# LY-zhang-yi-hao/ORB-SLAM3_byZyh

Measured on AMD Instinct MI355X. Metric: ORB features/ms (640x480, 8-level) + LocalBA iter ms @1/2/4/8 GPU, higher is better.
Workload: dtype u8; 1 GPU; C2: batch of 64 synthetic 640x480 frames per GPU, nFeatures=1000, 8 levels, extraction+description (ORBextractor::operator()); frames_per_gpu=64, width=640, height=480, nfeatures=1000, nlevels=8, batches_in_flight=4, parallelism=frame-sharded x1

## Files before the change

orb-slam3_byzyh_amd/csrc/orb_extract.hip:

```cpp
#include <hip/hip_ext.h>
#include <hip/hip_runtime.h>

#include <algorithm>
#include <cstdio>
#include <cstdlib>
#include <cstring>
#include <mutex>
#include <string>
#include <type_traits>
#include <vector>

#include "orb_extract_geom.h"
#include "orb_hd.h"
#include "orb_sincos.h"
#include "orbgpu.h"
#include "orbgpu_internal.h"

using namespace orbgpu;

namespace {

constexpr int kPatternSrc[1024] = {
#include "orb_pattern31.inc"
};
// ... 495 lines not shown
            const int r = r0o + lr;
            if (lr < rpp && r < nrow) {
                const int y = oy0 + r;
                const uint8_t* urow = ubuf + (reflect101(y, A.hl) - uy0) * kPairUP;
                uint8_t* dst = plane_l + (size_t)(y + kEdge) * A.pitch_l;
                const int pc = pc0 + 8 * ch, x = pc - kEdge;
                if (x >= ox0 && x + 8 <= ox1 && x >= 0 && x + 8 <= A.wl) {
                    *reinterpret_cast<unsigned long long*>(dst + pc) = lds_bytes8(urow, x - ux0);
                } else {
#pragma unroll
                    for (int b = 0; b < 8; ++b)
                        if (x + b >= ox0 && x + b < ox1) dst[pc + b] = urow[reflect101(x + b, A.wl) - ux0];
                }
            }
        }
    }
    {
        const int sx = XN.x - ux0, sx1 = min(XN.x + 1, ux0 + uw - 1) - ux0;
        pyr_resize_col<kTileH / 2>(ubuf, &yrowT[r0], sx, sx1, (unsigned)XN.y & 0xffffu, (unsigned)XN.y >> 16,
                                   vxn < A.simd_n, true, &tile[r0][tx], kTileW + 8);
    }
    __syncthreads();
#pragma unroll
    for (int r = tid >> 4; r < kTileH; r += 16) {
        const int c = (tid & 15) * 8;
        const int py = Y0 + r, px = X0 + c;
        if (py < ey && px < ex) {
            uint8_t* dst = plane_n + (size_t)py * A.pitch_n + px;
            if (px + 7 < ex) {
                *reinterpret_cast<unsigned long long*>(dst) = lds_bytes8(tile[r], c);
            } else {
                for (int k = 0; k < 8 && px + k < ex; ++k) dst[k] = tile[r][c + k];
            }
        }
    }
}

__global__ __launch_bounds__(256) void k_debug_blur(const uint8_t* __restrict__ view, int pitch, int w, int h,
                                                    uint8_t* __restrict__ out) {
    const int x = blockIdx.x * 256 + threadIdx.x, y = blockIdx.y;
    if (x >= w) return;
    uint32_t acc = 1u << 15;
    for (int i = 0; i < 7; ++i) {
        const uint8_t* row = view + (size_t)reflect101(y + i - 3, h) * pitch;
        uint32_t hs = 0;
        for (int k = 0; k < 7; ++k) hs += (uint32_t)(blur_tap(k) * row[reflect101(x + k - 3, w)]);
        acc += (uint32_t)blur_tap(i) * hs;
    }
    out[(size_t)y * w + x] = (uint8_t)(acc >> 16);
}

__device__ __forceinline__ u16x2 swap16(u16x2 a) { return __builtin_shufflevector(a, a, 1, 0); }
__device__ __forceinline__ int fast_score(const uint8_t* __restrict__ p, const int (&off)[16]) {
    const int v = p[0];
    const u16x2 vv = w16(v + 256, v + 256);
    u16x2 D[8];
#pragma unroll
    for (int k = 0; k < 8; ++k)
        D[k] = vv - __builtin_bit_cast(u16x2, (uint32_t)p[off[k]] | ((uint32_t)p[off[k + 8]] << 16));
    auto at = [&](const u16x2 (&a)[8], int k) { return k < 8 ? a[k] : swap16(a[k - 8]); };
    u16x2 mn2[8], mx2[8], mn4[8], mx4[8];
#pragma unroll
    for (int k = 0; k < 8; ++k) {
        mn2[k] = __builtin_elementwise_min(D[k], at(D, k + 1));
        mx2[k] = __builtin_elementwise_max(D[k], at(D, k + 1));
    }
#pragma unroll
    for (int k = 0; k < 8; ++k) {
        mn4[k] = __builtin_elementwise_min(mn2[k], at(mn2, k + 2));
        mx4[k] = __builtin_elementwise_max(mx2[k], at(mx2, k + 2));
    }
    u16x2 dark = w16(0, 0), bright = w16(0xffff, 0xffff);
#pragma unroll
    for (int k = 0; k < 8; ++k) {
        const u16x2 mn8 = __builtin_elementwise_min(mn4[k], at(mn4, k + 4));
        const u16x2 mx8 = __builtin_elementwise_max(mx4[k], at(mx4, k + 4));
        dark = __builtin_elementwise_max(dark, __builtin_elementwise_min(mn8, swap16(D[k])));
        bright = __builtin_elementwise_min(bright, __builtin_elementwise_max(mx8, swap16(D[k])));
    }
    const int best_dark = (int)max(dark.x, dark.y) - 256, best_bright = (int)min(bright.x, bright.y) - 256;
    return max(best_dark, -best_bright) - 1;
}

__device__ __forceinline__ bool is_local_max(const uint8_t* __restrict__ sc, int stride, int idx, int s) {
    const uint8_t* q = sc + idx;
    return s > q[-stride - 1] && s > q[-stride] && s > q[-stride + 1] && s > q[-1] && s > q[1] &&
           s > q[stride - 1] && s > q[stride] && s > q[stride + 1];
}

__device__ __forceinline__ uint32_t pack_key(int x, int y, int score) {
    return (uint32_t)score | ((uint32_t)x << 8) | ((uint32_t)y << 20);
}
__device__ __forceinline__ int key_x(uint32_t k) { return (int)((k >> 8) & 0xfff); }
__device__ __forceinline__ int key_y(uint32_t k) { return (int)(k >> 20); }
__device__ __forceinline__ int key_score(uint32_t k) { return (int)(k & 0xff); }

#define FAST_STAMP(k) do { if (stp && lane == 0) stp[k] = __builtin_amdgcn_s_memtime(); } while (0)
template <int kWS, int kSS>
__device__ __forceinline__ void fast_cell(const KernelGeom& g, const CellDesc& C, const LevelGeom& L, int f, int cid,
                                          int lane, uint8_t* win, uint8_t* sc, uint16_t* cl, const uint8_t* src,
                                          int shift, int room, uint32_t* __restrict__ cand, int32_t* __restrict__ cell_count,
                                          uint8_t* __restrict__ cell_thr, unsigned long long* stp) {
    const int ww = C.win_w, wh = C.win_h;
    const int ws = kWS ? kWS : (shift + ww + 3) & ~3, nwr = ws >> 2;
    const int ss = kSS ? kSS : (ww - 4 + 3) & ~3;
    auto sc_at = [&](int e) { return ((e >> 7) - 2) * ss + (e & 127) - 2; };
    const uint32_t* wsrc = reinterpret_cast<const uint32_t*>(src - shift);
    uint32_t* win32 = reinterpret_cast<uint32_t*>(win);
    const int lr = lane >> 4, lw = lane & 15;
    if (nwr <= 16 && wh <= 48) {
        const uintptr_t wb = reinterpret_cast<uintptr_t>(wsrc);
        const uint64_t wbu = (uint64_t)(uint32_t)uniform((int)(uint32_t)wb) | (uint64_t)(uint32_t)uniform((int)(uint32_t)(wb >> 32)) << 32;
        const __amdgpu_buffer_rsrc_t rw = __builtin_amdgcn_make_buffer_rsrc(reinterpret_cast<void*>(wbu), (short)0, uniform(room), kBufDword3);
        const int pitch = uniform(L.pitch);
        const uint32_t vo = (uint32_t)(lr * pitch + 4 * lw);
        uint32_t v[12];
#pragma unroll
        for (int k = 0; k < 12; ++k) v[k] = __builtin_amdgcn_raw_buffer_load_b32(rw, vo, 4 * k * pitch, 0);
#pragma unroll
        for (int k = 0; k < 12; ++k) {
            const int r = 4 * k + lr;
            if (r < wh && lw < nwr) win32[r * nwr + lw] = v[k];
        }
    } else
    for (int w0 = 0; w0 < nwr; w0 += 16) {
        const int w = w0 + lw;
        for (int r0 = 0; r0 < wh; r0 += 16) {
            uint32_t v[4];
#pragma unroll
            for (int k = 0; k < 4; ++k) {
                const int r = r0 + 4 * k + lr;
                v[k] = (r < wh && w < nwr) ? wsrc[(size_t)r * (L.pitch >> 2) + w] : 0u;
            }
#pragma unroll
            for (int k = 0; k < 4; ++k) {
                const int r = r0 + 4 * k + lr;
                if (r < wh && w < nwr) win32[r * nwr + w] = v[k];
            }
        }
    }
    wave_sync();
    FAST_STAMP(1);
    win += shift;
    const int dw = ww - 6, dh = wh - 6;
    const int nd = (dw > 0 && dh > 0) ? dw * dh : 0;
    int off[16];
    {
        const int cx[16] = {0, 1, 2, 3, 3, 3, 2, 1, 0, -1, -2, -3, -3, -3, -2, -1};
        const int cy[16] = {3, 3, 2, 1, 0, -1, -2, -3, -3, -3, -2, -1, 0, 1, 2, 3};
#pragma unroll
        for (int k = 0; k < 16; ++k) off[k] = cx[k] + cy[k] * ws;
    }
    const int ini = g.ini_th, mint = g.min_th;
    int nlist = 0;
    if (nd > 0) {
        const int no = (dw + 7) >> 3, nitems = dh * no;
        const uint32_t* wrow = reinterpret_cast<const uint32_t*>(win - shift);
        const int wsw = ws >> 2;
        const u16x2 tt = w16(mint, mint);
        auto ext8 = [&](const uint32_t* row, int o, int off, uint32_t& a, uint32_t& b) {
            const int d = 2 * o + (off >> 2);
            const uint32_t w0 = row[d], w1 = row[d + 1], w2 = row[d + 2];
            a = __builtin_amdgcn_alignbyte(w1, w0, off & 3);
            b = __builtin_amdgcn_alignbyte(w2, w1, off & 3);
        };
        auto lo16 = [](uint32_t v) { return as_u16x2(__builtin_amdgcn_perm(v, v, 0x0c010c00u)); };
        auto hi16 = [](uint32_t v) { return as_u16x2(__builtin_amdgcn_perm(v, v, 0x0c030c02u)); };
        auto pass2 = [&](u16x2 v, u16x2 p0, u16x2 p4, u16x2 p8, u16x2 p12) {
            const u16x2 bmax = __builtin_elementwise_min(__builtin_elementwise_max(p0, p8), __builtin_elementwise_max(p4, p12));
            const u16x2 dmin = __builtin_elementwise_max(__builtin_elementwise_min(p0, p8), __builtin_elementwise_min(p4, p12));
            const u16x2 m = __builtin_elementwise_max(__builtin_elementwise_sub_sat(bmax, v), __builtin_elementwise_sub_sat(v, dmin));
            uint32_t r;
            asm("v_pk_min_u16 %0, %1, %2" : "=v"(r) : "v"(__builtin_bit_cast(uint32_t, __builtin_elementwise_sub_sat(m, tt))), "v"(0x00010001u));
            return r;
        };
        auto octet_bits = [&](uint32_t C0, uint32_t D0, uint32_t R0, uint32_t U0, uint32_t L0, uint32_t C1,
                              uint32_t D1, uint32_t R1, uint32_t U1, uint32_t L1) {
            const uint32_t p01 = pass2(lo16(C0), lo16(D0), lo16(R0), lo16(U0), lo16(L0));
            const uint32_t p23 = pass2(hi16(C0), hi16(D0), hi16(R0), hi16(U0), hi16(L0));
            const uint32_t p45 = pass2(lo16(C1), lo16(D1), lo16(R1), lo16(U1), lo16(L1));
            const uint32_t p67 = pass2(hi16(C1), hi16(D1), hi16(R1), hi16(U1), hi16(L1));
            const uint32_t t = p01 | (p23 << 2) | (p45 << 4) | (p67 << 6);
            return (t & 0xffu) | (t >> 15);
        };
        int r = lane / no, o = lane - (lane / no) * no;
        const int dr = 64 / no, dq = 64 - dr * no;
        for (int i0 = 0; i0 < nitems; i0 += 64) {
            const int it = i0 + lane;
            unsigned bits = 0;
            if (it < nitems) {
                const uint32_t* rc = wrow + (r + 3) * wsw;
                uint32_t L0, L1, C0, C1, R0, R1, U0, U1, D0, D1;
                ext8(rc, o, shift, L0, L1);
                ext8(rc, o, shift + 3, C0, C1);
                ext8(rc, o, shift + 6, R0, R1);
                ext8(rc - 3 * wsw, o, shift + 3, U0, U1);
                ext8(rc + 3 * wsw, o, shift + 3, D0, D1);
                bits = octet_bits(C0, D0, R0, U0, L0, C1, D1, R1, U1, L1);
                const int rem = dw - 8 * o;
                if (rem < 8) bits &= (1u << rem) - 1u;
            }
            const int row = r, oct = o;
            o += dq;
            r += dr;
            if (o >= no) { o -= no; ++r; }
            const int cnt = __popc(bits);
            const int incl = wave_incl_scan_dpp(cnt);
            int pos = nlist + incl - cnt;
            const int base_idx = ((row + 3) << 7) + 8 * oct + 3;
            while (bits) {
                const int k = __builtin_ctz(bits);
                bits &= bits - 1u;
                cl[pos++] = (uint16_t)(base_idx + k);
            }
            nlist += __builtin_amdgcn_readlane(incl, 63);
        }
    }
    wave_sync();
    FAST_STAMP(2);
    int ncand = 0;
    for (int j0 = 0; j0 < nlist; j0 += 64) {
        const int j = j0 + lane;
        int idx = 0, s = -1;
        if (j < nlist) {
            idx = cl[j];
            s = fast_score(win + (idx >> 7) * ws + (idx & 127), off);
        }
        const bool is_c = s >= mint;
        const unsigned long long m = ballot(is_c);
        if (is_c) {
            cl[ncand + rank_in(m)] = (uint16_t)idx;
            sc[sc_at(idx)] = (uint8_t)min(s, 255);
        }
        ncand += __popcll(m);
    }
    wave_sync();
    FAST_STAMP(3);
    FAST_STAMP(4);
    uint8_t* lmv = win - shift;
    bool any = false;
    for (int j = lane; j < ncand; j += 64) {
        const int si = sc_at(cl[j]), s = sc[si];
        const bool lm = is_local_max(sc, ss, si, s);
        lmv[j] = lm ? (uint8_t)(s + 1) : (uint8_t)0;
        any |= (s >= ini) && lm;
    }
    const int t = ballot(any) ? ini : mint;
    wave_sync();
    FAST_STAMP(5);
    uint32_t* out = cand + (size_t)f * g.cand_frame_cap + L.cand_off + C.slot;
    int count = 0;
    for (int j0 = 0; j0 < ncand; j0 += 64) {
        const int j = j0 + lane;
        bool keep = false;
        int idx = 0, s = 0;
        if (j < ncand) {
            idx = cl[j];
            const int lv = lmv[j];
            s = lv - 1;
            keep = lv > 0 && s >= t;
        }
        const unsigned long long m = ballot(keep);
        if (keep) {
            const int pos = count + rank_in(m);
            const int r = idx >> 7, c = idx & 127;
            if (pos < C.cap) out[pos] = pack_key(C.off_x + c, C.off_y + r, s);
        }
        count += __popcll(m);
    }
    if (lane == 0) {
        cell_count[(size_t)f * g.ncells + cid] = min(count, (int)C.cap);
        cell_thr[(size_t)f * g.ncells + cid] = (uint8_t)t;
    }
    if (stp && lane == 0) { stp[6] = __builtin_amdgcn_s_memtime(); stp[8] = wall_clock64(); stp[9] = nlist; stp[10] = ncand; }
}


__global__ __launch_bounds__(256) void k_fast_cells(const KernelGeom* __restrict__ gp, const CellDesc* __restrict__ cells, int win_cap, int sc_cap, int wave_lds,
                                                    const uint8_t* __restrict__ pyr, uint32_t* __restrict__ cand,
                                                    int32_t* __restrict__ cell_count, uint8_t* __restrict__ cell_thr,
                                                    int cell0, int cell_end, unsigned long long* __restrict__ stamps,
                                                    int groups, int nblocks, int share) {
    const KernelGeom& g = *gp;
    extern __shared__ __attribute__((aligned(16))) uint8_t smem[];
    const int wave = threadIdx.x >> 6, lane = threadIdx.x & 63;
    const int tb = xcd_tile(blockIdx.x, share);
    if (tb >= nblocks) return;
    const int f = tb / groups;
    const int cid = cell0 + (tb - f * groups) * 4 + wave;
    if (cid >= cell_end) return;
    unsigned long long* stp = stamps ? stamps + ((size_t)f * (cell_end - cell0) + (cid - cell0)) * 12 : nullptr;
    if (stp && lane == 0) { stp[7] = wall_clock64(); stp[0] = __builtin_amdgcn_s_memtime(); }
    const CellDesc C = cells[cid];
    const LevelGeom& L = g.lv[C.level];
    const uint8_t* view = pyr + (size_t)f * g.pyr_frame_bytes + L.plane_off + (size_t)kEdge * L.pitch + kEdge;
    uint8_t* win = smem + (size_t)wave * wave_lds;
    uint8_t* sc = win + win_cap;
    uint16_t* cl = reinterpret_cast<uint16_t*>(sc + sc_cap);
    const uint8_t* src = view + (size_t)C.ini_y * L.pitch + C.ini_x;
    const int shift = (int)((uintptr_t)src & 3);
    const int room = (int)(g.pyr_frame_bytes - (L.plane_off + (long long)(kEdge + C.ini_y) * L.pitch + kEdge + C.ini_x - shift));
    for (int i = lane; i < (sc_cap >> 4); i += 64) reinterpret_cast<uint4*>(sc)[i] = make_uint4(0u, 0u, 0u, 0u);
    if (shift + C.win_w <= 52 && C.win_h <= 48) {
        if (C.win_w <= 44)
            fast_cell<52, 40>(g, C, L, f, cid, lane, win, sc, cl, src, shift, room, cand, cell_count, cell_thr, stp);
        else
            fast_cell<52, 48>(g, C, L, f, cid, lane, win, sc, cl, src, shift, room, cand, cell_count, cell_thr, stp);
    } else {
        fast_cell<0, 0>(g, C, L, f, cid, lane, win, sc, cl, src, shift, room, cand, cell_count, cell_thr, stp);
    }
}
#undef FAST_STAMP

struct QGen {
    int16_t *x0, *y0, *x1, *y1;
    int32_t* kn;
    uint8_t* leaf;
};

struct QTree {
    QGen g0, g1;
    uint16_t *split, *prev;
    uint8_t* divided;
    int* sort_ws;
    unsigned long long *sel_el, *sel_tmp;
    uint16_t *posA, *posB, *bend;
    int lcap;
};

__device__ __forceinline__ void split_point(const QGen& G, int p, int& sx, int& sy) {
    const int x0 = G.x0[p], y0 = G.y0[p], x1 = G.x1[p], y1 = G.y1[p];
    sx = x0 + ((x1 - x0 + 1) >> 1);
    sy = y0 + ((y1 - y0 + 1) >> 1);
}

__device__ __forceinline__ int wave_incl_scan(int v, int) { return wave_incl_scan_dpp(v); }

__device__ __forceinline__ int wave_incl_max(int v, int) { return wave_incl_max_dpp(v); }

__device__ void qt_sort(QTree& t, const QGen& A, int n, int lane) {
    unsigned long long* el = t.sel_el;
    auto less64 = [](unsigned long long x, unsigned long long y) { return (x >> 16) < (y >> 16); };
    for (int i = lane; i < n; i += 64) {
        const int id = t.prev[i];
        const uint32_t key = ((uint32_t)A.kn[id] << 16) | (uint16_t)A.x0[id];
        el[i] = ((unsigned long long)key << 16) | (unsigned)id;
        t.bend[i] = 0;
    }
    wave_sync();
    if (n <= 1) return;
    if (n > 16) {
        int lg = 0;
        for (int m = n; m > 1; m >>= 1) ++lg;
        int* st = t.sort_ws;
        if (lane == 0) { st[0] = 0; st[1] = n; st[2] = 2 * lg; }
        int sp = 1;
        wave_sync();
        while (sp > 0) {
            --sp;
            const int first = uniform(st[3 * sp]);
            int last = uniform(st[3 * sp + 1]), depth = uniform(st[3 * sp + 2]);
            while (last - first > 16) {
                if (depth == 0) {
                    if (lane == 0) orb_heap_sort(el, first, last, less64);
                    wave_sync();
                    break;
                }
                --depth;
                const int mid = first + (last - first) / 2;
                if (lane == 0) orb_move_median_to_first(el, first, first + 1, mid, last - 1, less64);
                wave_sync();
                const unsigned long long p = el[first] >> 16;
                int nA = 0, nB = 0;
                for (int b = first + 1; b < last; b += 64) {
                    const int i = b + lane;
                    const bool fa = i < last && !((el[i] >> 16) < p);
                    const unsigned long long m = ballot(fa);
                    if (fa) t.posA[nA + rank_in(m)] = (uint16_t)i;
                    nA += __popcll(m);
                }
                for (int b = last - 1; b > first; b -= 64) {
                    const int j = b - lane;
                    const bool fb = j > first && !(p < (el[j] >> 16));
                    const unsigned long long m = ballot(fb);
                    if (fb) t.posB[nB + rank_in(m)] = (uint16_t)j;
                    nB += __popcll(m);
                }
                wave_sync();
                const int lim = min(nA, nB);
                int ks = lim;
                for (int b = 0; b < lim; b += 64) {
                    const int k = b + lane;
                    const unsigned long long m = ballot(k < lim && t.posA[k] >= t.posB[k]);
                    if (m) { ks = b + __ffsll((long long)m) - 1; break; }
                }
                ks = uniform(ks);
                const int cut = uniform(min(ks < nA ? (int)t.posA[ks] : 1 << 30, ks > 0 ? (int)t.posB[ks - 1] : 1 << 30));
                for (int k = lane; k < ks; k += 64) {
                    const int ia = t.posA[k], ib = t.posB[k];
                    const unsigned long long ea = el[ia], eb = el[ib];
                    el[ia] = eb;
                    el[ib] = ea;
                }
                if (lane == 0) { st[3 * sp] = cut; st[3 * sp + 1] = last; st[3 * sp + 2] = depth; }
                sp++;
                wave_sync();
                last = cut;
            }
            if (lane == 0) t.bend[first] = (uint16_t)last;
            wave_sync();
        }
    } else {
        if (lane == 0) t.bend[0] = (uint16_t)n;
        wave_sync();
    }
    int carry = -1;
    for (int b = 0; b < n; b += 64) {
        const int i = b + lane;
        int v = (i < n && t.bend[i] != 0) ? i : -1;
        v = max(wave_incl_max(v, lane), carry);
        if (i < n) {
            const int s0 = v, e0 = t.bend[v];
            const unsigned long long ki = el[i] >> 16;
            int r = s0;
            for (int j = s0; j < e0; ++j) {
                const unsigned long long kj = el[j] >> 16;
                r += (kj < ki) || (kj == ki && j < i);
// ... 1039 lines not shown
                tab[2 * idx] = make_int4(ux0 | uw << 16, uy0 | uh << 16, cx0 | cw << 16, cy0 | chh << 16);
                tab[2 * idx + 1] = make_int4((ox0 & 0xffff) | ox1 << 16, (oy0 & 0xffff) | oy1 << 16, 0, 0);
            }
    }
    return true;
}

int prepare(Extractor* e, int w, int h, int n) {
    if (w != e->cur_w || h != e->cur_h) {
        if (e->cur_w >= 0 && hipDeviceSynchronize() != hipSuccess) return orbgpu_fail(ORB_ERR_DEVICE, "sync failed");
        orbgpu::Geometry g;
        if (!orbgpu::build_geometry(e->P, w, h, g)) return orbgpu_fail(ORB_ERR_ARG, "image too small for the pyramid/cell grid");
        for (int v = 0; v < 16; ++v)
            if (g.k.umax[v] != kDiscUmax[v]) return orbgpu_fail(ORB_ERR_INTERNAL, "umax differs from the IC_Angle disc table");
        e->geo = g;
        e->cur_w = w;
        e->cur_h = h;
        int rc;
        if ((rc = grow(e->d_cells, e->cells_cap, g.cells.size())) != ORB_OK) return rc;
        if ((rc = grow(e->d_xtab, e->xtab_cap, std::max<size_t>(1, g.xtab.size() / 2))) != ORB_OK) return rc;
        if ((rc = grow(e->d_ytab, e->ytab_cap, std::max<size_t>(1, g.ytab.size() / 4))) != ORB_OK) return rc;
        if (!e->d_geom && hipMalloc(&e->d_geom, sizeof(orbgpu::KernelGeom)) != hipSuccess)
            return orbgpu_fail(ORB_ERR_DEVICE, "hipMalloc failed");
        if (hipMemcpy(e->d_geom, &g.k, sizeof(orbgpu::KernelGeom), hipMemcpyHostToDevice) != hipSuccess ||
            hipMemcpy(e->d_cells, g.cells.data(), g.cells.size() * sizeof(orbgpu::CellDesc), hipMemcpyHostToDevice) != hipSuccess ||
            (!g.xtab.empty() && hipMemcpy(e->d_xtab, g.xtab.data(), g.xtab.size() * 4, hipMemcpyHostToDevice) != hipSuccess) ||
            (!g.ytab.empty() && hipMemcpy(e->d_ytab, g.ytab.data(), g.ytab.size() * 4, hipMemcpyHostToDevice) != hipSuccess))
            return orbgpu_fail(ORB_ERR_DEVICE, "table upload failed");
        std::vector<int4> tt;
        tile_tables(g.k, tt, e->tile_off);
        for (int l = 1; l < g.k.nlevels; ++l) {
            const bool small = 4 * g.k.lv[l - 1].w <= 5 * g.k.lv[l].w && 4 * g.k.lv[l - 1].h <= 5 * g.k.lv[l].h;
            const int bwmax = (small ? kSmallBoxW : kBoxW) - 3, bhmax = small ? kSmallBoxH : kBoxH;
            const int t1 = l + 1 < g.k.nlevels ? e->tile_off[l + 1] : (int)tt.size();
            for (int t = e->tile_off[l]; t < t1; ++t)
                if ((tt[t].y >> 16) > bwmax || (tt[t].z >> 16) > bhmax) {
                    e->cur_w = e->cur_h = -1;
                    e->geo_ok = false;
                    return orbgpu_fail(ORB_ERR_ARG, "pyramid level ratio above 2 (scale factor too large)");
                }
        }
        if ((rc = grow(e->d_tiletab, e->tiletab_cap, tt.size())) != ORB_OK) return rc;
        if (hipMemcpy(e->d_tiletab, tt.data(), tt.size() * sizeof(int4), hipMemcpyHostToDevice) != hipSuccess)
            return orbgpu_fail(ORB_ERR_DEVICE, "table upload failed");
        std::vector<int4> pt;
        e->pair_ok = pair_tables(g.k, tt, e->tile_off, pt);
        if (e->pair_ok) {
            if ((rc = grow(e->d_pairtab, e->pairtab_cap, pt.size())) != ORB_OK) return rc;
            if (hipMemcpy(e->d_pairtab, pt.data(), pt.size() * sizeof(int4), hipMemcpyHostToDevice) != hipSuccess)
                return orbgpu_fail(ORB_ERR_DEVICE, "table upload failed");
        }
        e->geo_ok = true;
        size_t meta = 0;
        for (int l = 0; l < g.k.nlevels; ++l) {
            const int lcap = g.k.lv[l].sel_cap + 64;
            meta = std::max(meta, (qt2_meta_bytes(lcap) + 15) & ~(size_t)15);
        }
        const size_t want = meta + (size_t)e->qt_key_room * 1024;
        if (meta > 160 * 1024) return orbgpu_fail(ORB_ERR_ARG, "nfeatures too large for the quad-tree LDS budget");
        e->qt_lds = (int)std::min<size_t>(want, 160 * 1024);
        if (hipFuncSetAttribute((const void*)k_quadtree_kp, hipFuncAttributeMaxDynamicSharedMemorySize, 160 * 1024) !=
            hipSuccess)
            return orbgpu_fail(ORB_ERR_DEVICE, "cannot raise the quad-tree LDS limit");
    }
    const orbgpu::KernelGeom& k = e->geo.k;
    int rc;
    if ((rc = grow(e->d_pyr, e->pyr_cap, (size_t)k.pyr_frame_bytes * n)) != ORB_OK) return rc;
    if ((rc = grow(e->d_cand, e->cand_cap, (size_t)k.cand_frame_cap * n)) != ORB_OK) return rc;
    if ((rc = grow(e->d_scratch, e->scratch_cap, (size_t)k.cand_frame_cap * n * 2)) != ORB_OK) return rc;
    if ((rc = grow(e->d_cell_count, e->cell_count_cap, (size_t)k.ncells * n)) != ORB_OK) return rc;
    if ((rc = grow(e->d_cell_thr, e->cell_thr_cap, (size_t)k.ncells * n)) != ORB_OK) return rc;
    if ((rc = grow(e->d_sel, e->sel_cap, (size_t)k.sel_frame_cap * n)) != ORB_OK) return rc;
    if ((rc = grow(e->d_dst, e->dst_cap, (size_t)k.sel_frame_cap * n)) != ORB_OK) return rc;
    if ((rc = grow(e->d_sel_count, e->selcount_cap, (size_t)k.nlevels * n)) != ORB_OK) return rc;
    if ((rc = grow(e->d_lap_count, e->lapcount_cap, (size_t)k.nlevels * n)) != ORB_OK) return rc;
    if (e->desc_split) {
        if ((rc = grow(e->d_st_kp, e->st_kp_cap, (size_t)k.sel_frame_cap * n)) != ORB_OK) return rc;
        if ((rc = grow(e->d_st_desc, e->st_desc_cap, (size_t)k.sel_frame_cap * n * 32)) != ORB_OK) return rc;
    }
    if ((k.debug_flags & 4) && (rc = grow(e->d_stamps, e->stamps_cap, (size_t)k.nlevels * n * kQtStamps)) != ORB_OK) return rc;
    return ORB_OK;
}

int launch_chunk(Extractor* e, int f0, const uint8_t* d_images, int n, int stride, size_t frame_stride, int lap0,
                 int lap1, orb_keypoint_t* d_kps, uint8_t* d_desc, int cap, int32_t* d_counts, hipStream_t st) {
    const orbgpu::Geometry& G = e->geo;
    const orbgpu::KernelGeom& k = G.k;
    hipEvent_t* ev = nullptr;
    if (e->profile == 1 || e->profile == 2) {
        const size_t need = (size_t)(e->ev_used + 1) * (orbgpu::kStages + 1);
        while (e->events.size() < need) {
            hipEvent_t x;
            if (hipEventCreate(&x) != hipSuccess) return orbgpu_fail(ORB_ERR_DEVICE, "hipEventCreate failed");
            e->events.push_back(x);
        }
        ev = &e->events[(size_t)e->ev_used * (orbgpu::kStages + 1)];
        e->ev_used++;
        e->frames_profiled += n;
    }
    auto mark = [&](int i) {
        if (ev && (e->profile == 1 || (e->profile == 2 && i <= 1))) hipEventRecord(ev[i], st);
    };
    uint8_t* pyr = e->d_pyr + (size_t)f0 * k.pyr_frame_bytes;
    uint32_t* cand = e->d_cand + (size_t)f0 * k.cand_frame_cap;
    uint32_t* scratch = e->d_scratch + (size_t)f0 * k.cand_frame_cap * 2;
    int32_t* ccount = e->d_cell_count + (size_t)f0 * k.ncells;
    uint8_t* cthr = e->d_cell_thr + (size_t)f0 * k.ncells;
    uint32_t* sel = e->d_sel + (size_t)f0 * k.sel_frame_cap;
    int32_t* dst = e->d_dst + (size_t)f0 * k.sel_frame_cap;
    int32_t* scount = e->d_sel_count + (size_t)f0 * k.nlevels;
    int32_t* lapc = e->d_lap_count + (size_t)f0 * k.nlevels;
    const uint8_t* imgs = d_images + (size_t)f0 * frame_stride;
    orb_keypoint_t* kps = d_kps + (size_t)f0 * cap;
    uint8_t* desc = d_desc + (size_t)f0 * cap * 32;
    int32_t* counts = d_counts + 2 * (size_t)f0;
    mark(0);
    const int split = (n > 1 && e->fast_split > 0 && e->fast_split < k.nlevels) ? e->fast_split : 0;
    const bool fast_stamps = e->fast_stamps;
    auto launch_events = [&](int kernel) -> hipEvent_t* {
        if (e->profile != 3 || e->pyr_ev_used + 2 > e->pyr_events.size()) return nullptr;
        hipEvent_t* pe = &e->pyr_events[e->pyr_ev_used];
        e->pyr_ev_kernel[e->pyr_ev_used / 2] = kernel;
        e->pyr_ev_used += 2;
        return pe;
    };
    auto launch_fast = [&](int l0, int l1, hipStream_t s2) {
        if (e->ablate & 4) return;
        const int c0 = k.lv[l0].cell_begin, c1 = k.lv[l1 - 1].cell_begin + k.lv[l1 - 1].cell_count;
        if (c1 <= c0) return;
        unsigned long long* stamps = nullptr;
        const size_t ns = (size_t)(c1 - c0) * n * 12;
        if (fast_stamps && hipMalloc(&stamps, ns * 8) == hipSuccess) (void)hipMemsetAsync(stamps, 0, ns * 8, s2);
        int mw = 0, md = 0, ms = 0;
        for (int l = l0; l < l1; ++l) {
            mw = std::max(mw, G.max_win_lv[l]);
            md = std::max(md, G.max_det_lv[l]);
            ms = std::max(ms, G.max_sc_lv[l]);
        }
        const int win_cap = (mw + 15) & ~15, sc_cap = (ms + 15) & ~15;
        const int wave_lds = win_cap + sc_cap + ((2 * md + 15) & ~15);
        const int groups = (c1 - c0 + 3) / 4, nblocks = groups * n, share = (nblocks + 7) / 8;
        if (hipEvent_t* pe = launch_events(kLaunchFast))
            hipExtLaunchKernelGGL(k_fast_cells, dim3(8 * share), dim3(256), 4 * wave_lds, s2, pe[0], pe[1], 0, e->d_geom,
                                  e->d_cells, win_cap, sc_cap, wave_lds, pyr, cand, ccount, cthr, c0, c1, stamps, groups, nblocks,
                                  share);
        else
            hipLaunchKernelGGL(k_fast_cells, dim3(8 * share), dim3(256), 4 * wave_lds, s2, e->d_geom, e->d_cells, win_cap,
                               sc_cap, wave_lds, pyr, cand, ccount, cthr, c0, c1, stamps, groups, nblocks, share);
        if (stamps) {
            std::vector<unsigned long long> h(ns);
            (void)hipStreamSynchronize(s2);
            (void)hipMemcpy(h.data(), stamps, ns * 8, hipMemcpyDeviceToHost);
            (void)hipFree(stamps);
            double ph[6] = {0}, life = 0, sv = 0, cn = 0;
            unsigned long long t0 = ~0ull, t1 = 0;
            size_t cnt = 0;
            for (size_t i = 0; i < ns; i += 12) {
                if (!h[i + 7]) continue;
                ++cnt;
                for (int q = 1; q <= 6; ++q) ph[q - 1] += (double)(h[i + q] - h[i + q - 1]);
                life += (double)(h[i + 8] - h[i + 7]);
                sv += (double)h[i + 9];
                cn += (double)h[i + 10];
                t0 = std::min(t0, h[i + 7]);
                t1 = std::max(t1, h[i + 8]);
            }
            fprintf(stderr, "fast-stamps L%d-%d cells %zu span %.1f us life %.2f us conc %.0f | stage %.0f compass %.0f full %.0f score %.0f thr %.0f emit %.0f cyc | surv %.1f corners %.1f\n",
                    l0, l1 - 1, cnt, (t1 - t0) * 0.01, life / cnt * 0.01, life / (double)(t1 - t0), ph[0] / cnt, ph[1] / cnt,
                    ph[2] / cnt, ph[3] / cnt, ph[4] / cnt, ph[5] / cnt, sv / cnt, cn / cnt);
        }
    };
    auto launch_qt = [&](int l0, int l1, hipStream_t s2) {
        if (l1 <= l0 || (e->ablate & 8)) return;
        unsigned long long* qst = e->d_stamps ? e->d_stamps + (size_t)f0 * k.nlevels * kQtStamps : nullptr;
        if (hipEvent_t* pe = launch_events(kLaunchQuadtree))
            hipExtLaunchKernelGGL(k_quadtree_kp, dim3(l1 - l0, n), dim3(kQtThreads), e->qt_lds, s2, pe[0], pe[1], 0,
                                  e->d_geom, e->d_cells, cand, ccount, scratch, sel, scount, e->qt_lds, e->d_status, qst,
                                  lap0, lap1, dst, lapc, l0);
        else
            hipLaunchKernelGGL(k_quadtree_kp, dim3(l1 - l0, n), dim3(kQtThreads), e->qt_lds, s2, e->d_geom, e->d_cells, cand,
                               ccount, scratch, sel, scount, e->qt_lds, e->d_status, qst, lap0, lap1, dst, lapc, l0);
    };
    bool desc_split = false;
    auto launch_desc = [&](int mode, int lim, hipStream_t s2) {
        if (e->ablate & 16) return;
        int chunks = 0;
        for (int l = 0; l < lim; ++l) chunks += (k.lv[l].sel_cap + kDescKpPerBlock - 1) / kDescKpPerBlock;
        const int total = chunks * n, share = (total + 7) / 8;
        orb_keypoint_t* skp = e->d_st_kp ? e->d_st_kp + (size_t)f0 * k.sel_frame_cap : nullptr;
        uint8_t* sdesc = e->d_st_desc ? e->d_st_desc + (size_t)f0 * k.sel_frame_cap * 32 : nullptr;
        if (hipEvent_t* pe = launch_events(kLaunchDescribe))
            hipExtLaunchKernelGGL(k_describe, dim3(8 * share), dim3(256), 0, s2, pe[0], pe[1], 0, e->d_geom, pyr, sel, scount,
                                  dst, lapc, cap, kps, desc, counts, chunks, total, share, split, mode, skp, sdesc);
        else
            hipLaunchKernelGGL(k_describe, dim3(8 * share), dim3(256), 0, s2, e->d_geom, pyr, sel, scount, dst, lapc, cap,
                               kps, desc, counts, chunks, total, share, split, mode, skp, sdesc);
    };
    const int chain_s = std::min(std::max(e->fast_split_cfg, 1), k.nlevels);
    const int chain_lds_split = (n > 1 && chain_s < k.nlevels) ? e->chain_fast_split : 0;
    desc_split = e->desc_split && split > 0 && !e->fast_per_level && e->d_st_kp;
    const bool qts = (e->qt_split || desc_split) && split > 0 && !e->fast_per_level;
    const bool pyr_stamps = e->pyr_stamps;
    auto level_done = [&](int l) {
        if (!split && chain_lds_split == 2 && l == chain_s - 1) {
            launch_fast(0, chain_s, st);
        } else if (split && l == split - 1) {
            hipEventRecord(e->split_ev[0], st);
            hipStreamWaitEvent(e->side, e->split_ev[0], 0);
            launch_fast(0, split, e->side);
            if (qts) launch_qt(0, split, e->side);
            if (desc_split) launch_desc(1, split, e->side);
            hipEventRecord(e->split_ev[1], e->side);
        } else if (split && l >= split && e->fast_per_level) {
            hipEventRecord(e->lvl_ev[l], st);
            hipStreamWaitEvent(e->side2, e->lvl_ev[l], 0);
            launch_fast(l, l + 1, e->side2);
        }
    };
    const bool pairs = e->pyr_pair && e->pair_ok && !pyr_stamps;
    for (int l = 0; l < k.nlevels; ++l) {
        if (pairs && (l & 1) == 0 && l + 1 < k.nlevels && (e->pyr_pair == 1 || l == 0)) {
            const orbgpu::LevelGeom &Ll = k.lv[l], &Ln = k.lv[l + 1];
            PairArgs A{};
            A.frame_bytes = k.pyr_frame_bytes;
            A.plane_l = Ll.plane_off;
            A.plane_n = Ln.plane_off;
            if (l > 0) {
                const orbgpu::LevelGeom& P = k.lv[l - 1];
                A.src_off = P.plane_off + (long long)kEdge * P.pitch + kEdge;
                A.spitch = P.pitch;
            }
            A.wl = Ll.w; A.hl = Ll.h; A.pitch_l = Ll.pitch; A.xtab_l = Ll.xtab_off; A.ytab_l = Ll.ytab_off; A.simd_l = Ll.simd_end;
            A.wn = Ln.w; A.hn = Ln.h; A.pitch_n = Ln.pitch; A.xtab_n = Ln.xtab_off; A.ytab_n = Ln.ytab_off; A.simd_n = Ln.simd_end;
            A.tab_off = e->tile_off[l + 1];
            A.tiles_per_frame = pyr_tiles_x(Ln) * pyr_tiles_y(Ln);
            A.share = (A.tiles_per_frame + 7) / 8;
            A.frame_affine = e->pyr_affine && n % 8 == 0;
            const dim3 grid(8 * A.share, n);
            hipEvent_t* pe = launch_events(kLaunchPyramid);
            auto go = [&](auto kern, auto... args) {
                if (e->ablate & (l == 0 ? 3 : 1)) return;
                if (pe) hipExtLaunchKernelGGL(kern, grid, dim3(256), 0, st, pe[0], pe[1], 0, args...);
                else hipLaunchKernelGGL(kern, grid, dim3(256), 0, st, args...);
            };
            if (l == 0)
                go(k_pyramid_pair<true>, A, imgs, (long long)frame_stride, stride, pyr, (const int2*)e->d_xtab,
                   (const int4*)e->d_ytab, (const int4*)e->d_tiletab, (const int4*)e->d_pairtab,
                   e->clear_status_l0 && f0 == 0 ? e->d_status : (int*)nullptr);
            else
                go(k_pyramid_pair<false>, A, (const uint8_t*)nullptr, 0LL, 0, pyr, (const int2*)e->d_xtab,
                   (const int4*)e->d_ytab, (const int4*)e->d_tiletab, (const int4*)e->d_pairtab, (int*)nullptr);
            level_done(l);
            level_done(l + 1);
            ++l;
            continue;
        }
        const orbgpu::LevelGeom& L = k.lv[l];
        PyrArgs A{};
        A.frame_bytes = k.pyr_frame_bytes;
        A.plane_off = L.plane_off;
        A.w = L.w; A.h = L.h; A.pw = L.pw; A.ph = L.ph; A.pitch = L.pitch;
        A.xtab_off = L.xtab_off; A.ytab_off = L.ytab_off; A.simd_end = L.simd_end;
        if (l > 0) {
            const orbgpu::LevelGeom& P = k.lv[l - 1];
            A.src_off = P.plane_off + (long long)kEdge * P.pitch + kEdge;
            A.sw = P.w; A.sh = P.h; A.spitch = P.pitch;
        }
        A.tab_off = e->tile_off[l];
        A.tiles_per_frame = pyr_tiles_x(L) * pyr_tiles_y(L);
        A.share = (A.tiles_per_frame + 7) / 8;
        A.frame_affine = e->pyr_affine && n % 8 == 0;
        const dim3 grid(8 * A.share, n);
        unsigned long long* stamps = nullptr;
        const size_t nblk = (size_t)grid.x * grid.y;
        if (pyr_stamps && hipMalloc(&stamps, sizeof(unsigned long long) * 8 * nblk) == hipSuccess)
            (void)hipMemsetAsync(stamps, 0, sizeof(unsigned long long) * 8 * nblk, st);
        hipEvent_t* pe = launch_events(kLaunchPyramid);
        auto go = [&](auto kern, auto... args) {
            if (e->ablate & (l == 0 ? 2 : 1)) return;
            if ((e->ablate & 32) && l >= 4) return;
            if ((e->ablate & 64) && l >= 1 && l < 4) return;
            if (pe) hipExtLaunchKernelGGL(kern, grid, dim3(256), 0, st, pe[0], pe[1], 0, args...);
            else hipLaunchKernelGGL(kern, grid, dim3(256), 0, st, args...);
        };
        const int2* xt = e->d_xtab;
        const int4* yt = e->d_ytab;
        const int4* tt = e->d_tiletab;
        if (l == 0)
            go(k_pyramid_level<true>, A, imgs, (long long)frame_stride, stride, pyr, xt, yt, tt, stamps,
               e->clear_status_l0 && f0 == 0 ? e->d_status : (int*)nullptr);
        else if (4 * k.lv[l - 1].w <= 5 * L.w && 4 * k.lv[l - 1].h <= 5 * L.h)
            go(k_pyramid_level<false, kSmallBoxH, kSmallBoxW>, A, (const uint8_t*)nullptr, 0LL, 0, pyr, xt, yt, tt, stamps,
               (int*)nullptr);
        else
            go(k_pyramid_level<false, kBoxH, kBoxW>, A, (const uint8_t*)nullptr, 0LL, 0, pyr, xt, yt, tt, stamps,
               (int*)nullptr);
        if (stamps && pyr_stamps) {
            std::vector<unsigned long long> hst((size_t)8 * nblk);
            (void)hipStreamSynchronize(st);
            (void)hipMemcpy(hst.data(), stamps, hst.size() * 8, hipMemcpyDeviceToHost);
            (void)hipFree(stamps);
            double ph[4] = {0}, life = 0;
            unsigned long long t0 = ~0ull, t1 = 0;
            int cnt = 0;
            for (size_t b = 0; b < nblk; ++b) {
                const unsigned long long* q = &hst[(size_t)8 * b];
                if (!q[6]) continue;
                ++cnt;
                for (int i = 1; i < 4; ++i) ph[i] += (double)(q[i] - q[i - 1]);
                life += (double)(q[7] - q[6]);
                t0 = std::min(t0, q[6]);
                t1 = std::max(t1, q[7]);
            }
            fprintf(stderr, "pyr-stamps L%d blocks %d span %.1f us  mean life %.2f us  concurrency %.0f  phases(cyc) box %.0f resize %.0f store %.0f\n",
                    l, cnt, (t1 - t0) * 0.01, life / cnt * 0.01, life / (double)(t1 - t0), ph[1] / cnt, ph[2] / cnt,
                    ph[3] / cnt);
        }
        level_done(l);
    }
    mark(1);
    if (split && e->fast_per_level) {
        hipEventRecord(e->split_ev[2], e->side2);
// ... 508 lines not shown
```

orb-slam3_byzyh_amd/csrc/orb_extract_geom.h:

```cpp
#pragma once
#include <cmath>
#include <cstdlib>
#include <cstdint>
#include <vector>

namespace orbgpu {

constexpr int kMaxLevels = 12;
constexpr int kEdge = 19;
constexpr int kHalfPatch = 15;
constexpr int kPatchSize = 31;
constexpr int kCellW = 35;
constexpr int kMaxRoots = 8;
constexpr int kStages = 5;

struct LevelGeom {
    int w, h;
    int pw, ph, pitch;
    long long plane_off;
    int minB, maxBX, maxBY;
    int cell_begin, cell_count;
    int cand_off, cand_cap;
    int nfeat;
    int sel_off, sel_cap;
// ... 29 lines not shown
    int nfeatures = 0, nlevels = 0, ini_th = 0, min_th = 0;
    double scale_factor = 0;
    std::vector<float> scale, inv_scale, sigma2, inv_sigma2;
    std::vector<int> per_level, umax;
};

inline int round_half_even(float v) { return (int)std::lrintf(v); }
inline int floor_f(float v) { int i = (int)v; return i - (i > v); }
inline int ceil_f(float v) { int i = (int)v; return i + (i < v); }

inline Params make_params(int nfeatures, float scale_factor, int nlevels, int ini_th, int min_th) {
    Params p;
    p.nfeatures = nfeatures; p.nlevels = nlevels; p.ini_th = ini_th; p.min_th = min_th;
    p.scale_factor = scale_factor;
    p.scale.assign(nlevels, 1.0f);
    p.sigma2.assign(nlevels, 1.0f);
    for (int i = 1; i < nlevels; ++i) {
        p.scale[i] = (float)(p.scale[i - 1] * p.scale_factor);
        p.sigma2[i] = p.scale[i] * p.scale[i];
    }
    p.inv_scale.resize(nlevels);
    p.inv_sigma2.resize(nlevels);
    for (int i = 0; i < nlevels; ++i) {
        p.inv_scale[i] = 1.0f / p.scale[i];
        p.inv_sigma2[i] = 1.0f / p.sigma2[i];
    }
    const float factor = (float)(1.0f / p.scale_factor);
    float per_scale = nfeatures * (1 - factor) / (1 - (float)std::pow((double)factor, (double)nlevels));
    int sum = 0;
    p.per_level.assign(nlevels, 0);
    for (int l = 0; l < nlevels - 1; ++l) {
        p.per_level[l] = round_half_even(per_scale);
        sum += p.per_level[l];
        per_scale *= factor;
    }
    p.per_level[nlevels - 1] = std::max(nfeatures - sum, 0);
    p.umax.assign(kHalfPatch + 1, 0);
    const int vmax = floor_f(kHalfPatch * std::sqrt(2.f) / 2 + 1);
    const int vmin = ceil_f(kHalfPatch * std::sqrt(2.f) / 2);
    const double r2 = kHalfPatch * kHalfPatch;
    for (int v = 0; v <= vmax; ++v) p.umax[v] = (int)std::lrint(std::sqrt(r2 - v * v));
    for (int v = kHalfPatch, v0 = 0; v >= vmin; --v) {
        while (p.umax[v0] == p.umax[v0 + 1]) ++v0;
        p.umax[v] = v0;
        ++v0;
    }
    return p;
}

struct Geometry {
    KernelGeom k{};
    std::vector<CellDesc> cells;
    std::vector<int32_t> xtab;
    std::vector<int32_t> ytab;
    int max_win = 0;
    int max_win_lv[kMaxLevels] = {};
    int max_det_lv[kMaxLevels] = {};
    int max_sc_lv[kMaxLevels] = {};
    int max_level_cands = 0;
    int max_sel = 0;
};

inline int sat16(int v) { return v < -32768 ? -32768 : v > 32767 ? 32767 : v; }

inline void resize_tables(int sw, int sh, int dw, int dh, std::vector<int32_t>& xt, std::vector<int32_t>& yt) {
    const double scale_x = 1. / ((double)dw / sw), scale_y = 1. / ((double)dh / sh);
    for (int dx = 0; dx < dw; ++dx) {
        float fx = (float)((dx + 0.5) * scale_x - 0.5);
        int sx = floor_f(fx);
        fx -= sx;
        if (sx < 0) { fx = 0; sx = 0; }
        if (sx >= sw - 1) { fx = 0; sx = sw - 1; }
        const int a0 = sat16(round_half_even((1.f - fx) * 2048));
        const int a1 = sat16(round_half_even(fx * 2048));
        xt.push_back(sx);
        xt.push_back((a0 & 0xffff) | (a1 << 16));
    }
    for (int dy = 0; dy < dh; ++dy) {
        float fy = (float)((dy + 0.5) * scale_y - 0.5);
        const int sy = floor_f(fy);
        fy -= sy;
        const int b0 = sat16(round_half_even((1.f - fy) * 2048));
        const int b1 = sat16(round_half_even(fy * 2048));
        const int r0 = std::min(std::max(sy, 0), sh - 1), r1 = std::min(std::max(sy + 1, 0), sh - 1);
        yt.push_back(r0); yt.push_back(r1); yt.push_back(b0); yt.push_back(b1);
    }
}

inline int align_up(long long v, int a) { return (int)((v + a - 1) / a * a); }

inline bool build_geometry(const Params& P, int width, int height, Geometry& g) {
    g = Geometry();
    KernelGeom& k = g.k;
    k.nlevels = P.nlevels;
    k.ini_th = std::min(std::max(P.ini_th, 0), 255);
    k.min_th = std::min(std::max(P.min_th, 0), 255);
    k.debug_flags = 0;
    if (const char* d = getenv("ORBGPU_DEBUG_FLAGS")) k.debug_flags = atoi(d);
    for (int v = 0; v <= kHalfPatch; ++v) k.umax[v] = P.umax[v];
    long long plane_off = 0;
    int cand_off = 0, sel_off = 0;
    int prev_w = width, prev_h = height;
    for (int l = 0; l < P.nlevels; ++l) {
        LevelGeom& L = k.lv[l];
        L.w = round_half_even((float)width * P.inv_scale[l]);
        L.h = round_half_even((float)height * P.inv_scale[l]);
        if (L.w < 2 * kEdge || L.h < 2 * kEdge) return false;
        L.pw = L.w + 2 * kEdge;
        L.ph = L.h + 2 * kEdge;
        L.pitch = align_up(L.pw, 128);
        L.plane_off = plane_off;
        plane_off += (long long)L.pitch * L.ph;
        plane_off = (plane_off + 255) / 256 * 256;
        L.scale = P.scale[l];
        L.patch_size = (int)(kPatchSize * P.scale[l]);
        L.nfeat = P.per_level[l];
        L.minB = kEdge - 3;
        L.maxBX = L.w - kEdge + 3;
        L.maxBY = L.h - kEdge + 3;
        const float wid = (float)(L.maxBX - L.minB), hei = (float)(L.maxBY - L.minB);
        const int ncols = (int)(wid / kCellW), nrows = (int)(hei / kCellW);
        if (ncols <= 0 || nrows <= 0) return false;
        const int wcell = (int)std::ceil(wid / ncols), hcell = (int)std::ceil(hei / nrows);
        L.cell_begin = (int)g.cells.size();
        L.cand_off = cand_off;
        int level_cap = 0;
        for (int i = 0; i < nrows; ++i) {
            const float ini_y = (float)(L.minB + i * hcell);
            float max_y = ini_y + hcell + 6;
            if (ini_y >= L.maxBY - 3) continue;
            if (max_y > L.maxBY) max_y = (float)L.maxBY;
            for (int j = 0; j < ncols; ++j) {
                const float ini_x = (float)(L.minB + j * wcell);
                float max_x = ini_x + wcell + 6;
                if (ini_x >= L.maxBX - 6) continue;
                if (max_x > L.maxBX) max_x = (float)L.maxBX;
                CellDesc c{};
                c.level = (int16_t)l;
                c.ini_x = (int16_t)ini_x;
                c.ini_y = (int16_t)ini_y;
                c.win_w = (int16_t)((int)max_x - (int)ini_x);
                c.win_h = (int16_t)((int)max_y - (int)ini_y);
                c.off_x = (int16_t)(j * wcell);
                c.off_y = (int16_t)(i * hcell);
                const int dw = std::max(0, c.win_w - 6), dh = std::max(0, c.win_h - 6);
                c.cap = ((dw + 1) / 2) * ((dh + 1) / 2);
                c.slot = level_cap;
                level_cap += c.cap;
                const int wbytes = std::max((int)c.win_w + 6, 52) * c.win_h;
                g.max_win = std::max(g.max_win, wbytes);
                g.max_win_lv[l] = std::max(g.max_win_lv[l], wbytes);
                g.max_det_lv[l] = std::max(g.max_det_lv[l], dw * dh);
                if (c.win_w >= 128 || c.win_h >= 512) return false;
                const int ss = c.win_w <= 44 ? 40 : std::max(48, (c.win_w - 4 + 3) & ~3);
                g.max_sc_lv[l] = std::max(g.max_sc_lv[l], std::max(0, c.win_h - 4) * ss);
                g.cells.push_back(c);
            }
        }
        L.cell_count = (int)g.cells.size() - L.cell_begin;
        L.cand_cap = level_cap;
        cand_off += level_cap;
        g.max_level_cands = std::max(g.max_level_cands, level_cap);
        const int spanx = L.maxBX - L.minB, spany = L.maxBY - L.minB;
        L.n_roots = (int)std::round((float)spanx / spany);
        if (L.n_roots <= 0 || L.n_roots > kMaxRoots) return false;
        L.root_w = (float)spanx / L.n_roots;
        L.sel_cap = std::max(L.nfeat + 2, 4 * L.n_roots) + 2;
        L.sel_off = sel_off;
        sel_off += L.sel_cap;
        g.max_sel = std::max(g.max_sel, L.sel_cap);
        if (l > 0) {
            L.xtab_off = (int)g.xtab.size() / 2;
            L.ytab_off = (int)g.ytab.size() / 4;
            resize_tables(prev_w, prev_h, L.w, L.h, g.xtab, g.ytab);
            int x = 0;
            for (; x <= L.w - 16; x += 16) {}
            for (; x < L.w - 8; x += 8) {}
            L.simd_end = x;
        }
        prev_w = L.w;
        prev_h = L.h;
    }
    k.ncells = (int)g.cells.size();
    k.pyr_frame_bytes = plane_off;
    k.cand_frame_cap = cand_off;
    k.sel_frame_cap = sel_off;
    return true;
}

}
```

Measured before the change: 342,800 features/ms.

## Prefilter FAST candidates at the high threshold first, fall back to min threshold lazily

The pixel prefilter now computes pass bits for both the initial and the minimum FAST threshold in one pass. Full scoring and non-max suppression run first on the initial-threshold list only. The minimum-threshold bits are parked in registers so the candidate list can be rebuilt, with scores cleared, only when a cell yields no corners. This aims to avoid scoring the larger min-threshold candidate set in most cells and merges the threshold and emit phases, at the cost of a second full pass in fallback cells, extra registers, and a new geometry limit on octet items per cell.

```diff
diff --git a/orb-slam3_byzyh_amd/csrc/orb_extract.hip b/orb-slam3_byzyh_amd/csrc/orb_extract.hip
--- a/orb-slam3_byzyh_amd/csrc/orb_extract.hip
+++ b/orb-slam3_byzyh_amd/csrc/orb_extract.hip
@@ -671,127 +671,148 @@
         for (int k = 0; k < 16; ++k) off[k] = cx[k] + cy[k] * ws;
     }
     const int ini = g.ini_th, mint = g.min_th;
+    constexpr int kParkWords = kWS ? 1 : 4;
+    uint32_t parked[kParkWords] = {};
+    const int no = nd > 0 ? (dw + 7) >> 3 : 1, nitems = nd > 0 ? dh * no : 0;
+    const int r0 = lane / no, o0 = lane - r0 * no, dr = 64 / no, dq = 64 - dr * no;
+    auto next_item = [&](int& r, int& o) {
+        o += dq;
+        r += dr;
+        if (o >= no) { o -= no; ++r; }
+    };
     int nlist = 0;
-    if (nd > 0) {
-        const int no = (dw + 7) >> 3, nitems = dh * no;
+    auto append = [&](unsigned bits, int row, int oct) {
+        const int cnt = __popc(bits);
+        const int incl = wave_incl_scan_dpp(cnt);
+        int pos = nlist + incl - cnt;
+        const int base_idx = ((row + 3) << 7) + 8 * oct + 3;
+        while (bits) {
+            const int k = __builtin_ctz(bits);
+            bits &= bits - 1u;
+            cl[pos++] = (uint16_t)(base_idx + k);
+        }
+        nlist += __builtin_amdgcn_readlane(incl, 63);
+    };
+    {
         const uint32_t* wrow = reinterpret_cast<const uint32_t*>(win - shift);
         const int wsw = ws >> 2;
-        const u16x2 tt = w16(mint, mint);
-        auto ext8 = [&](const uint32_t* row, int o, int off, uint32_t& a, uint32_t& b) {
+        const u16x2 tmin = w16(mint, mint), tini = w16(ini, ini);
+        struct Sel { uint32_t s01, s23; };
+        auto sel = [&](int off) {
+            const int s = (off & 3) * 0x00010001;
+            return Sel{(uint32_t)uniform(0x0c010c00 + s), (uint32_t)uniform(0x0c030c02 + s)};
+        };
+        const Sel selL = sel(shift), selC = sel(shift + 3), selR = sel(shift + 6);
+        auto ext8 = [&](const uint32_t* row, int o, int off, const Sel& S, u16x2 (&p)[4]) {
             const int d = 2 * o + (off >> 2);
             const uint32_t w0 = row[d], w1 = row[d + 1], w2 = row[d + 2];
-            a = __builtin_amdgcn_alignbyte(w1, w0, off & 3);
-            b = __builtin_amdgcn_alignbyte(w2, w1, off & 3);
+            p[0] = as_u16x2(__builtin_amdgcn_perm(w1, w0, S.s01));
+            p[1] = as_u16x2(__builtin_amdgcn_perm(w1, w0, S.s23));
+            p[2] = as_u16x2(__builtin_amdgcn_perm(w2, w1, S.s01));
+            p[3] = as_u16x2(__builtin_amdgcn_perm(w2, w1, S.s23));
         };
-        auto lo16 = [](uint32_t v) { return as_u16x2(__builtin_amdgcn_perm(v, v, 0x0c010c00u)); };
-        auto hi16 = [](uint32_t v) { return as_u16x2(__builtin_amdgcn_perm(v, v, 0x0c030c02u)); };
         auto pass2 = [&](u16x2 v, u16x2 p0, u16x2 p4, u16x2 p8, u16x2 p12) {
             const u16x2 bmax = __builtin_elementwise_min(__builtin_elementwise_max(p0, p8), __builtin_elementwise_max(p4, p12));
             const u16x2 dmin = __builtin_elementwise_max(__builtin_elementwise_min(p0, p8), __builtin_elementwise_min(p4, p12));
             const u16x2 m = __builtin_elementwise_max(__builtin_elementwise_sub_sat(bmax, v), __builtin_elementwise_sub_sat(v, dmin));
-            uint32_t r;
-            asm("v_pk_min_u16 %0, %1, %2" : "=v"(r) : "v"(__builtin_bit_cast(uint32_t, __builtin_elementwise_sub_sat(m, tt))), "v"(0x00010001u));
-            return r;
+            uint32_t a, b;
+            asm("v_pk_min_u16 %0, %1, %2" : "=v"(a) : "v"(__builtin_bit_cast(uint32_t, __builtin_elementwise_sub_sat(m, tmin))), "v"(0x00010001u));
+            asm("v_pk_min_u16 %0, %1, %2" : "=v"(b) : "v"(__builtin_bit_cast(uint32_t, __builtin_elementwise_sub_sat(m, tini))), "v"(0x00010001u));
+            return a | (b << 8);
         };
-        auto octet_bits = [&](uint32_t C0, uint32_t D0, uint32_t R0, uint32_t U0, uint32_t L0, uint32_t C1,
-                              uint32_t D1, uint32_t R1, uint32_t U1, uint32_t L1) {
-            const uint32_t p01 = pass2(lo16(C0), lo16(D0), lo16(R0), lo16(U0), lo16(L0));
-            const uint32_t p23 = pass2(hi16(C0), hi16(D0), hi16(R0), hi16(U0), hi16(L0));
-            const uint32_t p45 = pass2(lo16(C1), lo16(D1), lo16(R1), lo16(U1), lo16(L1));
-            const uint32_t p67 = pass2(hi16(C1), hi16(D1), hi16(R1), hi16(U1), hi16(L1));
-            const uint32_t t = p01 | (p23 << 2) | (p45 << 4) | (p67 << 6);
-            return (t & 0xffu) | (t >> 15);
-        };
-        int r = lane / no, o = lane - (lane / no) * no;
-        const int dr = 64 / no, dq = 64 - dr * no;
-        for (int i0 = 0; i0 < nitems; i0 += 64) {
-            const int it = i0 + lane;
-            unsigned bits = 0;
-            if (it < nitems) {
+        int r = r0, o = o0;
+        for (int i0 = 0, k = 0; i0 < nitems; i0 += 64, ++k) {
+            unsigned both = 0;
+            if (i0 + lane < nitems) {
                 const uint32_t* rc = wrow + (r + 3) * wsw;
-                uint32_t L0, L1, C0, C1, R0, R1, U0, U1, D0, D1;
-                ext8(rc, o, shift, L0, L1);
-                ext8(rc, o, shift + 3, C0, C1);
-                ext8(rc, o, shift + 6, R0, R1);
-                ext8(rc - 3 * wsw, o, shift + 3, U0, U1);
-                ext8(rc + 3 * wsw, o, shift + 3, D0, D1);
-                bits = octet_bits(C0, D0, R0, U0, L0, C1, D1, R1, U1, L1);
+                u16x2 pl[4], pc[4], pr[4], pu[4], pd[4];
+                ext8(rc, o, shift, selL, pl);
+                ext8(rc, o, shift + 3, selC, pc);
+                ext8(rc, o, shift + 6, selR, pr);
+                ext8(rc - 3 * wsw, o, shift + 3, selC, pu);
+                ext8(rc + 3 * wsw, o, shift + 3, selC, pd);
+                const uint32_t t = pass2(pc[0], pd[0], pr[0], pu[0], pl[0]) | (pass2(pc[1], pd[1], pr[1], pu[1], pl[1]) << 2) |
+                                   (pass2(pc[2], pd[2], pr[2], pu[2], pl[2]) << 4) | (pass2(pc[3], pd[3], pr[3], pu[3], pl[3]) << 6);
+                both = (t | (t >> 15)) & 0xffffu;
                 const int rem = dw - 8 * o;
-                if (rem < 8) bits &= (1u << rem) - 1u;
-            }
-            const int row = r, oct = o;
-            o += dq;
-            r += dr;
-            if (o >= no) { o -= no; ++r; }
-            const int cnt = __popc(bits);
-            const int incl = wave_incl_scan_dpp(cnt);
-            int pos = nlist + incl - cnt;
-            const int base_idx = ((row + 3) << 7) + 8 * oct + 3;
-            while (bits) {
-                const int k = __builtin_ctz(bits);
-                bits &= bits - 1u;
-                cl[pos++] = (uint16_t)(base_idx + k);
-            }
-            nlist += __builtin_amdgcn_readlane(incl, 63);
+                if (rem < 8) both &= 0x0101u * ((1u << rem) - 1u);
+            }
+#pragma unroll
+            for (int q = 0; q < kParkWords; ++q)
+                if (kParkWords == 1 || (k >> 2) == q) parked[q] |= (both & 0xffu) << (8 * (k & 3));
+            append(both >> 8, r, o);
+            next_item(r, o);
         }
     }
     wave_sync();
     FAST_STAMP(2);
-    int ncand = 0;
-    for (int j0 = 0; j0 < nlist; j0 += 64) {
-        const int j = j0 + lane;
-        int idx = 0, s = -1;
-        if (j < nlist) {
-            idx = cl[j];
-            s = fast_score(win + (idx >> 7) * ws + (idx & 127), off);
-        }
-        const bool is_c = s >= mint;
-        const unsigned long long m = ballot(is_c);
-        if (is_c) {
-            cl[ncand + rank_in(m)] = (uint16_t)idx;
-            sc[sc_at(idx)] = (uint8_t)min(s, 255);
-        }
-        ncand += __popcll(m);
-    }
-    wave_sync();
-    FAST_STAMP(3);
-    FAST_STAMP(4);
-    uint8_t* lmv = win - shift;
-    bool any = false;
-    for (int j = lane; j < ncand; j += 64) {
-        const int si = sc_at(cl[j]), s = sc[si];
-        const bool lm = is_local_max(sc, ss, si, s);
-        lmv[j] = lm ? (uint8_t)(s + 1) : (uint8_t)0;
-        any |= (s >= ini) && lm;
-    }
-    const int t = ballot(any) ? ini : mint;
-    wave_sync();
-    FAST_STAMP(5);
     uint32_t* out = cand + (size_t)f * g.cand_frame_cap + L.cand_off + C.slot;
-    int count = 0;
-    for (int j0 = 0; j0 < ncand; j0 += 64) {
-        const int j = j0 + lane;
-        bool keep = false;
-        int idx = 0, s = 0;
-        if (j < ncand) {
-            idx = cl[j];
-            const int lv = lmv[j];
-            s = lv - 1;
-            keep = lv > 0 && s >= t;
-        }
-        const unsigned long long m = ballot(keep);
-        if (keep) {
-            const int pos = count + rank_in(m);
-            const int r = idx >> 7, c = idx & 127;
-            if (pos < C.cap) out[pos] = pack_key(C.off_x + c, C.off_y + r, s);
-        }
-        count += __popcll(m);
+    int t = ini, count = 0, ncand = 0, scored = 0, rounds = 0;
+    for (;;) {
+        ncand = 0;
+        for (int j0 = 0; j0 < nlist; j0 += 64) {
+            const int j = j0 + lane;
+            int idx = 0, s = -1;
+            if (j < nlist) {
+                idx = cl[j];
+                s = fast_score(win + (idx >> 7) * ws + (idx & 127), off);
+            }
+            const bool is_c = s >= t;
+            const unsigned long long m = ballot(is_c);
+            if (is_c) {
+                cl[ncand + rank_in(m)] = (uint16_t)idx;
+                sc[sc_at(idx)] = (uint8_t)min(s, 255);
+            }
+            ncand += __popcll(m);
+        }
+        scored += nlist;
+        rounds += (nlist + 63) >> 6;
+        wave_sync();
+        FAST_STAMP(3);
+        count = 0;
+        for (int j0 = 0; j0 < ncand; j0 += 64) {
+            const int j = j0 + lane;
+            bool keep = false;
+            int idx = 0, s = 0;
+            if (j < ncand) {
+                idx = cl[j];
+                const int si = sc_at(idx);
+                s = sc[si];
+                keep = is_local_max(sc, ss, si, s);
+            }
+            const unsigned long long m = ballot(keep);
+            if (keep) {
+                const int pos = count + rank_in(m);
+                const int r = idx >> 7, c = idx & 127;
+                if (pos < C.cap) out[pos] = pack_key(C.off_x + c, C.off_y + r, s);
+            }
+            count += __popcll(m);
+        }
+        if (count > 0 || t == mint) break;
+        wave_sync();
+        for (int j = lane; j < ncand; j += 64) sc[sc_at(cl[j])] = 0;
+        wave_sync();
+        nlist = 0;
+        int r = r0, o = o0;
+        for (int i0 = 0, k = 0; i0 < nitems; i0 += 64, ++k) {
+            unsigned bits = 0;
+#pragma unroll
+            for (int q = 0; q < kParkWords; ++q)
+                if (kParkWords == 1 || (k >> 2) == q) bits = (parked[q] >> (8 * (k & 3))) & 0xffu;
+            append(bits, r, o);
+            next_item(r, o);
+        }
+        wave_sync();
+        t = mint;
     }
     if (lane == 0) {
         cell_count[(size_t)f * g.ncells + cid] = min(count, (int)C.cap);
         cell_thr[(size_t)f * g.ncells + cid] = (uint8_t)t;
     }
-    if (stp && lane == 0) { stp[6] = __builtin_amdgcn_s_memtime(); stp[8] = wall_clock64(); stp[9] = nlist; stp[10] = ncand; }
+    if (stp && lane == 0) {
+        stp[4] = __builtin_amdgcn_s_memtime(); stp[8] = wall_clock64();
+        stp[5] = t != ini; stp[6] = rounds; stp[9] = scored; stp[10] = ncand;
+    }
 }
 
 
@@ -2137,22 +2158,24 @@
             (void)hipStreamSynchronize(s2);
             (void)hipMemcpy(h.data(), stamps, ns * 8, hipMemcpyDeviceToHost);
             (void)hipFree(stamps);
-            double ph[6] = {0}, life = 0, sv = 0, cn = 0;
+            double ph[4] = {0}, life = 0, sv = 0, cn = 0, fb = 0, rd = 0;
             unsigned long long t0 = ~0ull, t1 = 0;
             size_t cnt = 0;
             for (size_t i = 0; i < ns; i += 12) {
                 if (!h[i + 7]) continue;
                 ++cnt;
-                for (int q = 1; q <= 6; ++q) ph[q - 1] += (double)(h[i + q] - h[i + q - 1]);
+                for (int q = 1; q <= 4; ++q) ph[q - 1] += (double)(h[i + q] - h[i + q - 1]);
+                fb += (double)h[i + 5];
+                rd += (double)h[i + 6];
                 life += (double)(h[i + 8] - h[i + 7]);
                 sv += (double)h[i + 9];
                 cn += (double)h[i + 10];
                 t0 = std::min(t0, h[i + 7]);
                 t1 = std::max(t1, h[i + 8]);
             }
-            fprintf(stderr, "fast-stamps L%d-%d cells %zu span %.1f us life %.2f us conc %.0f | stage %.0f compass %.0f full %.0f score %.0f thr %.0f emit %.0f cyc | surv %.1f corners %.1f\n",
+            fprintf(stderr, "fast-stamps L%d-%d cells %zu span %.1f us life %.2f us conc %.0f | stage %.0f compass %.0f score %.0f emit %.0f cyc | scored %.1f corners %.1f rounds %.3f minTh cells %.4f\n",
                     l0, l1 - 1, cnt, (t1 - t0) * 0.01, life / cnt * 0.01, life / (double)(t1 - t0), ph[0] / cnt, ph[1] / cnt,
-                    ph[2] / cnt, ph[3] / cnt, ph[4] / cnt, ph[5] / cnt, sv / cnt, cn / cnt);
+                    ph[2] / cnt, ph[3] / cnt, sv / cnt, cn / cnt, rd / cnt, fb / cnt);
         }
     };
     auto launch_qt = [&](int l0, int l1, hipStream_t s2) {
diff --git a/orb-slam3_byzyh_amd/csrc/orb_extract_geom.h b/orb-slam3_byzyh_amd/csrc/orb_extract_geom.h
--- a/orb-slam3_byzyh_amd/csrc/orb_extract_geom.h
+++ b/orb-slam3_byzyh_amd/csrc/orb_extract_geom.h
@@ -205,6 +205,7 @@
                 g.max_win_lv[l] = std::max(g.max_win_lv[l], wbytes);
                 g.max_det_lv[l] = std::max(g.max_det_lv[l], dw * dh);
                 if (c.win_w >= 128 || c.win_h >= 512) return false;
+                if ((dw + 7) / 8 * dh > 1024) return false;
                 const int ss = c.win_w <= 44 ? 40 : std::max(48, (c.win_w - 4 + 3) & ~3);
                 g.max_sc_lv[l] = std::max(g.max_sc_lv[l], std::max(0, c.win_h - 4) * ss);
                 g.cells.push_back(c);
```

Measured after the change: 363,100 features/ms, median of 6. +5.9%, better.
